# CaNS-World/CaLES

Measured on AMD Instinct MI355X. Metric: time-steps/sec, higher is better.
Workload: dtype f64; 1 GPU; turbulent channel 512x512x512, sgstype=dsmag, PP/PP/NN pressure BCs, bulk forcing in x (BASELINE.json configs[2]); 3 RK substeps/step; decomposition=single GPU

## Files before the change

cales_amd/csrc/api.hip:

```cpp
#include "common.hpp"

static thread_local std::string g_create_err;

void launch_failed(cales_ctx *c, const char *what, hipError_t e) {
  if (c->launch_err.empty()) c->launch_err = std::string("kernel launch failed: ") + what + ": " + hipGetErrorString(e) + " (the context is unusable from here on)";
}
static int finish_pending(cales_ctx *c);
#define ENTER(c) do { LAUNCHCHK(c); if (const int pe_ = finish_pending(c)) return pe_; } while (0)
#define ENTRY(c, expr) do { ENTER(c); const int e_ = (expr); if (e_) return e_; LAUNCHCHK(c); return 0; } while (0)

int stream_after(cales_ctx *c, hipStream_t later, hipStream_t earlier) {
  if (c->sync_ev.size() < 64) { hipEvent_t e; HIPCHK(c, hipEventCreateWithFlags(&e, hipEventDisableTiming)); c->sync_ev.push_back(e); c->sync_next = c->sync_ev.size() - 1; }
  hipEvent_t e = c->sync_ev[c->sync_next]; c->sync_next = (c->sync_next + 1) % c->sync_ev.size();
  HIPCHK(c, hipEventRecord(e, earlier));
  HIPCHK(c, hipStreamWaitEvent(later, e, 0));
  return 0;
}
int prof_begin(cales_ctx *c, const char *name, hipStream_t s) {
  int slot = -1;
  for (size_t q = 0; q < c->stats.size(); ++q) if (c->stats[q].name == name) { slot = (int)q; break; }
  if (slot < 0) { KernelStat s; s.name = name; c->stats.push_back(s); slot = (int)c->stats.size() - 1; }
  std::pair<hipEvent_t, hipEvent_t> ev;
  if (!c->evpool.empty()) { ev = c->evpool.back(); c->evpool.pop_back(); }
  else { hipEventCreate(&ev.first); hipEventCreate(&ev.second); }
  hipEventRecord(ev.first, s ? s : c->stream);
  c->pending.push_back({slot, ev});
  return (int)c->pending.size() - 1;
}
void prof_end(cales_ctx *c, int idx, hipStream_t s) { hipEventRecord(c->pending[idx].second.second, s ? s : c->stream); }
void prof_flush(cales_ctx *c) {
  if (c->pending.empty()) return;
  hipStreamSynchronize(c->stream);
  if (c->comm_stream) hipStreamSynchronize(c->comm_stream);
  for (auto &pe : c->pending) {
    float ms = 0.f;
    hipEventElapsedTime(&ms, pe.second.first, pe.second.second);
    c->stats[pe.first].calls += 1; c->stats[pe.first].ms += ms;
    c->evpool.push_back(pe.second);
  }
  c->pending.clear();
}

static int dev_alloc(cales_ctx *c, real **p, size_t n, bool zero = true) {
  HIPCHK(c, hipMalloc(p, (n ? n : 1) * sizeof(real)));
  if (zero) HIPCHK(c, hipMemset(*p, 0, (n ? n : 1) * sizeof(real)));
  return 0;
}
static int field_alloc(cales_ctx *c, real **p) {
  real *base = nullptr;
  if (dev_alloc(c, &base, c->ntot + LINE_REALS)) return 1;
  *p = base + c->field_ofs;
  return 0;
}
static void field_free(cales_ctx *c, real *p) { if (p) hipFree(p - c->field_ofs); }
static int field_alloc_multi(cales_ctx *c, int k, real **p) {
  real *base = nullptr;
  const size_t one = c->ntot + LINE_REALS;
  if (dev_alloc(c, &base, (size_t)k * one)) return 1;
  for (int q = 0; q < k; ++q) p[q] = base + (size_t)q * one + c->field_ofs;
  c->pp_companion_bytes = one * sizeof(real); c->comp_one = one;
  return 0;
// ... 106 lines not shown
  for (int d = 0; d < 3; ++d) { c->dl[d] = cs->l[d] / (real)(1.f * (float)cs->ng[d]); c->dli[d] = 1. / c->dl[d]; }
  c->visc = 1. / cs->visci;
  Geom &g = c->g;
  g.n1 = c->n[0]; g.n2 = c->n[1]; g.n3 = c->n[2];
  g.s1 = (g.n1 + 3 + LINE_REALS - 1) / LINE_REALS * LINE_REALS;
  c->field_ofs = LINE_REALS - 1;
  g.s12 = (long)g.s1 * (g.n2 + 2); g.jlo = c->lo[1] - 1; g.ng2 = cs->ng[1];
  c->ntot = (size_t)g.s12 * (g.n3 + 2);
  const int n3 = c->n[2];
  c->dzc.resize(n3 + 2); c->dzf.resize(n3 + 2); c->zc.resize(n3 + 2); c->zf.resize(n3 + 2);
  c->dzci.resize(n3 + 2); c->dzfi.resize(n3 + 2); c->gvr_c.resize(n3 + 2); c->gvr_f.resize(n3 + 2);
  hs_initgrid(cs->gtype, n3, cs->gr, cs->l[2], c->dzc.data(), c->dzf.data(), c->zc.data(), c->zf.data());
  for (int k = 0; k <= n3 + 1; ++k) {
    c->dzci[k] = 1. / c->dzc[k]; c->dzfi[k] = 1. / c->dzf[k];
    c->gvr_c[k] = c->dl[0] * c->dl[1] * c->dzc[k] / (cs->l[0] * cs->l[1] * cs->l[2]);
    c->gvr_f[k] = c->dl[0] * c->dl[1] * c->dzf[k] / (cs->l[0] * cs->l[1] * cs->l[2]);
  }
  if (upload_vec(c, &c->d_dzc, c->dzc) || upload_vec(c, &c->d_dzf, c->dzf) || upload_vec(c, &c->d_zc, c->zc) || upload_vec(c, &c->d_zf, c->zf) ||
      upload_vec(c, &c->d_dzci, c->dzci) || upload_vec(c, &c->d_dzfi, c->dzfi) || upload_vec(c, &c->d_gvr_c, c->gvr_c) || upload_vec(c, &c->d_gvr_f, c->gvr_f))
    return fail(5);
  c->is_bound[0] = c->is_bound[1] = 1;
  { c->is_bound[2] = (!c->per_y && r == 0) ? 1 : 0; c->is_bound[3] = (!c->per_y && r == P - 1) ? 1 : 0;
    const bool per_z = cs->cbcpre[4] == 'P' && cs->cbcpre[5] == 'P';
    c->is_bound[4] = c->is_bound[5] = per_z ? 0 : 1; }
  std::vector<real> hb[11][3];
  hs_initbc(c, hb);
  for (int q = 0; q < 11; ++q) if (upload_bound(c, *bs[q], hb[q])) return fail(6);
  for (int d = 1; d <= 3; ++d) for (int s = 0; s <= 1; ++s) c->is_wall[s + 2 * (d - 1)] = (ISB(c, s, d) && CBV(c, s, d, d) == 'D') ? 1. : 0.;
  for (int s = 0; s <= 1; ++s) c->is_wall[s + 2] = (!c->per_y && CBV(c, s, 2, 2) == 'D') ? 1. : 0.;
  sgs_setup(c);
  bc_setup(c);
  { const int *n = c->n;
    const real dx01[2] = {c->dl[0], c->dl[0]}, dy01[2] = {c->dl[1], c->dl[1]};
    const real dzc01[2] = {c->dzc[0], c->dzc[n3]}, dzf01[2] = {c->dzf[1], c->dzf[n3]};
    std::vector<real> rx((size_t)n[1] * n[2] * 2), ry((size_t)n[0] * n[2] * 2), rz((size_t)n[0] * n[1] * 2);
    hs_bc_rhs(&cs->cbcpre[0], hb[3][0].data(), n[1], n[2], dx01, dx01, 'c', rx.data());
    hs_bc_rhs(&cs->cbcpre[2], hb[3][1].data(), n[0], n[2], dy01, dy01, 'c', ry.data());
    hs_bc_rhs(&cs->cbcpre[4], hb[3][2].data(), n[0], n[1], dzc01, dzf01, 'c', rz.data());
    if (upload_vec(c, &c->rhsbp[0], rx) || upload_vec(c, &c->rhsbp[1], ry) || upload_vec(c, &c->rhsbp[2], rz)) return fail(7); }
  const int nfields = cs->impdiff ? CALES_NFIELDS : CALES_DUDTD;
  c->vel_comp = P > 1 && fold_correc_possible(c) && c->n[1] >= 4 && 3 * (c->ntot + 2 * LINE_REALS) * sizeof(real) < (1ull << 32) && !c->fl.unmerged_bc;
  for (int q = 0; q < nfields; ++q) {
    if (q == CALES_PP) continue;
    if (c->vel_comp && q <= CALES_W) { real *two[2]; if (field_alloc_multi(c, 2, two)) return fail(8); c->f[q] = two[0]; }
    else if (field_alloc(c, &c->f[q])) return fail(8);
  }
  { real *three[3]; if (field_alloc(c, &c->scr1) || field_alloc_multi(c, c->vel_comp ? 3 : 2, three)) return fail(9);
    c->f[CALES_PP] = three[0]; c->scr2 = three[1]; c->scr3 = c->vel_comp ? three[2] : nullptr; }
  for (int q = 0; q < 3; ++q) {
    if (c->vel_comp) { real *two[2]; if (field_alloc_multi(c, 2, two)) return fail(9); c->f2[q] = two[0]; }
    else if (field_alloc(c, &c->f2[q])) return fail(9);
  }
  c->red_blocks = 8;
  if (dev_alloc(c, &c->d_red, 64 + 16 * (size_t)(n3 + 2) + 6 * (size_t)(n3 + 2)) || dev_alloc(c, &c->d_force, 8)) return fail(10);
  c->res = c->d_red;
  if (hipHostMalloc((void **)&c->h_red, 64 * sizeof(real)) != hipSuccess) { c->err = "hipHostMalloc failed"; return fail(11); }
  if (cs->sgstype >= 1) {
    if (field_alloc(c, &c->s0)) return fail(12);
    const int nw = cs->sgstype == 1 ? 3 : 6;
    for (int m = 0; m < nw; ++m) if (field_alloc(c, &c->wk[m])) return fail(12);
  }
  if (cs->sgstype == 2) {
    if (field_alloc(c, &c->uc) || field_alloc(c, &c->vc) || field_alloc(c, &c->wc) || field_alloc(c, &c->uf) ||
        field_alloc(c, &c->vf) || field_alloc(c, &c->wf) || field_alloc(c, &c->alph2) || dev_alloc(c, &c->d_p1d, 2 * (size_t)n3 + 2))
      return fail(13);
    if (c->sgs.pair) {
      for (int m = 0; m < 3; ++m) { real *b = nullptr; if (dev_alloc(c, &b, 2 * c->ntot + 2 * LINE_REALS)) return fail(13); c->ss2[m] = b + 2 * c->field_ofs; }
    } else
    for (int m = 0; m < 6; ++m) if (field_alloc(c, &c->sij[m]) || field_alloc(c, &c->mij[m])) return fail(13);
  }
  if (solver_setup(c)) return fail(14);
  { hipDeviceProp_t pr; int dev = 0; if (hipGetDevice(&dev) == hipSuccess && hipGetDeviceProperties(&pr, dev) == hipSuccess) c->ncu = pr.multiProcessorCount; }
  if (sgs_setup_launches(c)) return fail(14);
  mom_setup(c);
  if (hipStreamSynchronize(c->stream) != hipSuccess) { c->err = "sync failed"; return fail(15); }
  if (!c->launch_err.empty()) { c->err = c->launch_err; return fail(16); }
  *out = c;
  return 0;
}

int cales_sync(cales_ctx *c) { ENTER(c); HIPCHK(c, hipStreamSynchronize(c->stream)); return 0; }
int cales_local_size(const cales_ctx *c, int32_t n[3], int32_t lo[3]) { for (int d = 0; d < 3; ++d) { n[d] = c->n[d]; lo[d] = c->lo[d]; } return 0; }

int cales_set_field(cales_ctx *c, int field, const real *host) {
  ENTER(c);
  if (field < 0 || field >= CALES_NFIELDS || !c->f[field]) { c->err = "bad field id"; return 1; }
  if (field == CALES_VISCT) { c->visct_zero = false; c->visct_lazy = false; }
  const size_t nh = (size_t)(c->n[0] + 2) * (c->n[1] + 2) * (c->n[2] + 2);
  const dim3 b(64, 4, 1), gr((c->n[0] + 2 + 63) / 64, (c->n[1] + 2 + 3) / 4, c->n[2] + 2);
  HIPCHK(c, hipMemcpyAsync(c->scr1, host, nh * sizeof(real), hipMemcpyHostToDevice, c->stream));
  LAUNCH(c, k_repack, gr, b, 0, c->stream, c->g, 1, c->f[field], c->scr1);
  LAUNCHCHK(c);
  HIPCHK(c, hipStreamSynchronize(c->stream));
  return 0;
}
int cales_get_field(cales_ctx *c, int field, real *host) {
  ENTER(c);
  if (field < 0 || field >= CALES_NFIELDS || !c->f[field]) { c->err = "bad field id"; return 1; }
  if (field == CALES_VISCT) if (int e = materialize_visct(c)) return e;
  const size_t nh = (size_t)(c->n[0] + 2) * (c->n[1] + 2) * (c->n[2] + 2);
  const dim3 b(64, 4, 1), gr((c->n[0] + 2 + 63) / 64, (c->n[1] + 2 + 3) / 4, c->n[2] + 2);
  LAUNCH(c, k_repack, gr, b, 0, c->stream, c->g, 0, c->f[field], c->scr1);
  LAUNCHCHK(c);
  HIPCHK(c, hipMemcpyAsync(host, c->scr1, nh * sizeof(real), hipMemcpyDeviceToHost, c->stream));
  HIPCHK(c, hipStreamSynchronize(c->stream));
  return 0;
}
// ... 144 lines not shown
  pl.any_wm = any_wm(c);
  pl.fuse_fill = fuse_fill_possible(c) && solver_can_fuse_fillps(c);
  pl.xskip = pl.fuse_fill && xskip_possible(c);
  pl.fold_correc = pl.xskip && fold_correc_possible(c) && (c->P == 1 || c->comm.on);
  pl.fold_rows2 = pl.fold_correc && c->vel_comp;
  pl.fold_mom = !pl.fold_correc && fold_mom_ok(c);
  pl.lazy_last = pl.fold_mom && !fl.eager_projection && c->P == 1 && (fl.lazy_projection || (size_t)c->n[0] * c->n[1] * c->n[2] >= ((size_t)1 << 22));
  { const char *bz = &c->cbcvel[4];
    pl.defer_imp_rhs = c->C.impdiff == 2 && !fl.helmholtz_z_per_column && !fl.unfused_imp_rhs &&
                       !(bz[0] == 'P' && bz[1] == 'P') && !(bz[6] == 'P' && bz[7] == 'P') && !(bz[12] == 'P' && bz[13] == 'P'); }
  { bool dead = !wm_samples_ghost(c);
    for (int sd = 0; sd <= 1; ++sd) if (LWM(c, sd, 1) != 0) dead = false;
    pl.skip_first_wm = dead && pl.any_wm && !fl.unmerged_bc; }
  pl.fuse_cu = fuse_cu_possible(c);
  { bool ok = c->C.impdiff == 0 && pl.fuse_cu && !fl.unfused_forcing && (!pl.any_wm || pl.skip_first_wm);
    for (int d = 0; d < 3; ++d) if (c->C.is_forced[d]) ok = ok && c->cbcvel[6 * d + 2 * d] == 'P' && c->cbcvel[6 * d + 2 * d + 1] == 'P';
    pl.force_mask = (c->C.is_forced[0] ? 1 : 0) | (c->C.is_forced[1] ? 2 : 0) | (c->C.is_forced[2] ? 4 : 0);
    pl.defer_force = ok && pl.force_mask != 0; }
  pl.mean_mask = (pl.fuse_fill && pl.defer_force && !fl.unfused_mean) ? pl.force_mask : 0;
  pl.keep_last_rhs = fl.keep_last_rhs;
  pl.visct_ghosts = !(c->C.sgstype == 0 && (c->visct_zero || c->sgs_first));
  for (int q = 0; q < 6; ++q) if (c->C.bcsgs[q] != 0.) pl.visct_ghosts = true;
  c->plan = pl;
}
static const StepPlan &current_plan(cales_ctx *c) {
  const StepPlan &pl = c->plan;
  if (!pl.valid || pl.in_visct_zero != c->visct_zero || pl.in_sgs_first != c->sgs_first || pl.in_comm_on != c->comm.on || pl.in_overlap != (c->comm_stream != nullptr)) make_plan(c);
  return c->plan;
}
int cales_describe_plan(cales_ctx *c, char *buf, int buflen) {
  if (!c || !buf || buflen < 1) return 1;
  const StepPlan &pl = current_plan(c);
  std::string s;
  s += std::string("projection=") + (pl.fold_rows2 ? "in_strain_rate_pass(ghost_rows_local)" : pl.fold_correc ? "in_strain_rate_pass" : pl.fold_mom ? (pl.lazy_last ? "in_next_momentum_pass(all_substeps)" : "in_next_momentum_pass(substeps_1_2)") : (pl.fuse_cu ? "own_pass(correc+updatep)" : "own_passes"));
  s += std::string(";x_ghost_columns=") + (pl.xskip ? "wrapped" : "maintained");
  s += std::string(";fillps=") + (pl.fuse_fill ? "in_x_transform" : "own_pass");
  s += std::string(";bulk_forcing=") + (pl.force_mask == 0 ? "none" : pl.defer_imp_rhs ? "in_helmholtz_sweep" : pl.defer_force ? (pl.mean_mask ? "in_correction(means_in_x_transform)" : "in_correction(means_own_pass)") : "own_pass");
  if (c->C.impdiff == 2) s += std::string(";implicit_rhs=") + (pl.defer_imp_rhs ? "in_helmholtz_sweep" : "own_pass");
  if (pl.any_wm) s += std::string(";first_wall_model_update=") + (pl.skip_first_wm ? "skipped" : "kept");
  s += std::string(";ghost_cells=") + (c->fl.unmerged_bc ? "by_direction" : "one_launch");
  s += std::string(";visct_ghost_cells=") + (pl.visct_ghosts ? "updated" : "zero_field");
  s += std::string(";momentum=") + (c->mom.fused ? "fused_mom_rk" : "mom+rk_update");
  s += std::string(";sgs=") + sgs_path_name(c);
  s += std::string(";solver=") + solver_path_name(c);
  if (c->P > 1) s += ";mode_columns_per_rank=" + std::to_string(solver_mode_columns(c));
  s += ";ranks=" + std::to_string(c->P) + ";exchanges=" + (c->P == 1 ? "none" : !c->comm.on ? "unset" : (c->comm_stream && (c->comm.halo_s || c->comm.a2a_part)) ? "second_stream" : "in_order");
  std::snprintf(buf, buflen, "%s", s.c_str());
  return (int)s.size() < buflen ? 0 : 2;
}

static int step_body(cales_ctx *c, real dt);
int cales_step(cales_ctx *c, real dt) {
  LAUNCHCHK(c);
  const int e = step_body(c, dt);
  LAUNCHCHK(c);
  if (e) { c->launch_err = "an earlier cales_step failed (" + c->err + "): the fields are in an intermediate state, the context is unusable"; return e; }
  return 0;
}
static int step_body(cales_ctx *c, real dt) {
  static const real rk[3][2] = {{32. / 60., 0.}, {25. / 60., -17. / 60.}, {45. / 60., -25. / 60.}};
  const StepPlan pl = current_plan(c);
  if (c->pend.dtrk != 0. && !pl.fold_mom) { if (int e = finish_pending(c)) return e; }
  PendingProjection pend = c->pend;
  c->pend = PendingProjection();
  LAUNCH(c, k_zero6, dim3(1), dim3(64), 0, c->stream, c->d_force, pend.dtrk != 0. ? 3 : 0);
  c->in_step = true;
  StepMode mode{c};
  if (c->pend_xrefresh && !pl.xskip) {
    c->pend_xrefresh = false; c->step_xskip = true;
    if (int e = end_of_step_refresh(c)) return e;
  }
  c->step_xskip = pl.xskip;
  const int fmask = pl.defer_force ? pl.force_mask : 0;
  SgsFold fold{0., pl.fold_rows2, fmask};
  for (int irk = 1; irk <= 3; ++irk) {
    const real dtrk = (rk[irk - 1][0] + rk[irk - 1][1]) * dt, dtrki = 1. / dtrk;
    real alpha = 0.;
    const bool p_ghosts_due = pend.dtrk != 0. && !pend.p_done;
    { RkOpts o; o.mean_mask = pl.mean_mask; o.rhs_in_sweep = pl.defer_imp_rhs; o.store_rhs = irk < 3 || pl.keep_last_rhs; o.pending = pend.dtrk != 0. ? &pend : nullptr;
      if (int e = op_rk(c, irk, dt, o)) return e;
      pend = PendingProjection(); }
    if (!pl.defer_force && !pl.defer_imp_rhs) { if (int e = op_bulk_forcing(c)) return e; }
    if (c->C.impdiff == 2) {
      alpha = -.5 * c->visc * dtrk;
      const real hf12 = .5 * (rk[irk - 1][0] * dt + rk[irk - 1][1] * dt);
      for (int iv = 1; iv <= 3; ++iv) if (int e = op_helmholtz_z(c, iv, alpha, pl.defer_imp_rhs, hf12)) return e;
    } else if (c->C.impdiff == 1) {
      alpha = -.5 * c->visc * dtrk;
      for (int iv = 1; iv <= 3; ++iv) if (int e = op_helmholtz(c, iv, alpha)) return e;
    }
    { BcCall b; b.skip_wm = pl.skip_first_wm;
      if (p_ghosts_due) b.rider(c->f[CALES_P], 0);
      HaloBatch rows; if (pl.fold_rows2) b.collect = &rows;
      if (int e = op_bounduvw(c, c->bcu, c->bcv, c->bcw, 1, 0, c->f[CALES_U], c->f[CALES_V], c->f[CALES_W], b)) return e;
      if (pl.fold_rows2) {
        if (int e = halo_y_rows(c, 3, c->f + CALES_U, 2, b)) return e;
        if (int e = halo_flush_deferred(c, rows, false)) return e;
      } }
    if (!pl.fuse_fill) { if (int e = op_fillps(c, dtrki)) return e; if (int e = op_updt_rhs_b(c)) return e; }
    if (int e = op_solver(c, pl.fuse_fill ? FusedFill{dtrki, pl.mean_mask} : FusedFill())) return e;
    if (pl.fold_rows2) {
      HaloBatch rows; BcCall b; b.collect = &rows;
      real *one[1] = {c->f[CALES_PP]};
      if (int e = op_boundp(c, c->f[CALES_PP], 0, b)) return e;
      if (int e = halo_y_rows(c, 1, one, 2, b)) return e;
      if (int e = halo_y_rows(c, 1, one, 3, b)) return e;
// ... 128 lines not shown
```

cales_amd/csrc/common.hpp:

```cpp
#pragma once
#include <hip/hip_runtime.h>
#include <cstdint>
#include <cstdio>
#include <cstdlib>
#include <cstring>
#include <cmath>
#include <string>
#include <vector>
#include "../../include/cales.h"

typedef cales_real real;
#ifdef CALES_SINGLE
typedef float2 real2;
#define CALES_EPS 1.1920929e-07f
#define CALES_BIG 3.4028235e38f
#else
typedef double2 real2;
#define CALES_EPS 2.220446049250313e-16
#define CALES_BIG 1.7976931348623157e308
#endif
constexpr int RSZ = (int)sizeof(real);
constexpr int LINE_REALS = 128 / RSZ;
__host__ __device__ inline real2 make_real2(real x, real y) { real2 r; r.x = x; r.y = y; return r; }

struct Geom {
  int n1, n2, n3;
  int s1;
  long s12;
  int jlo;
  int ng2;

  __host__ __device__ inline size_t ix(int i, int j, int k) const { return (size_t)i + (size_t)s1 * (size_t)j + (size_t)s12 * (size_t)k; }
};

struct DBound { real *x, *y, *z; };
struct RhsBz {
  const real *bc; char ctype, cf; real dlc, dlf, sgn, alpha;
  __host__ __device__ inline real at(int i, int j, int n1) const {
    const real bcv = bc[i + (size_t)(n1 + 2) * j];
    real r = 0.;
    if (cf == 'c') { if (ctype == 'D') r = -2. * bcv / dlc / dlf; else if (ctype == 'N') r = sgn * bcv / dlf; }
    else           { if (ctype == 'D') r = -bcv / dlc / dlf;      else if (ctype == 'N') r = sgn * bcv / dlc; }
    return r * alpha;
  }
};

struct Comm {
  cales_halo_cb halo = nullptr; cales_alltoall_cb a2a = nullptr; cales_allreduce_cb allred = nullptr; void *user = nullptr;
  real *A = nullptr, *B = nullptr; int64_t nbuf = 0;
  bool on = false;
  cales_halo_s_cb halo_s = nullptr; cales_alltoall_part_cb a2a_part = nullptr;
};

struct Spec {
  int blocked, cw, n2l, n3;
  int nyq = 0;
  __host__ __device__ inline size_t at_slab(const Geom &g, int m, int jl, int k) const {
    if (!blocked) return (g.ix(0, jl, k) >> 1) + (size_t)m;
    const int peer = m / cw, mm = m - peer * cw;
    return (size_t)mm + (size_t)cw * ((size_t)(jl - 1) + (size_t)n2l * ((size_t)(k - 1) + (size_t)n3 * peer));
  }
  __host__ __device__ inline size_t at_mode(const Geom &g, int mm, int j, int k) const {
    if (!blocked) return (g.ix(0, j, k) >> 1) + (size_t)mm;
    const int peer = (j - 1) / n2l, jl = (j - 1) - peer * n2l;
    return (size_t)mm + (size_t)cw * ((size_t)jl + (size_t)n2l * ((size_t)(k - 1) + (size_t)n3 * peer));
  }
};

struct Flags {
  bool unfolded_correc = false, unfolded_mom = false, eager_projection = false, lazy_projection = false, helmholtz_z_per_column = false, unfused_imp_rhs = false, unfused_correc = false, unfused_forcing = false, unfused_fillps = false, unfused_mean = false, keep_last_rhs = false, wide_offsets = false, dsmag_reference_sequence = false, dsmag_xghosts = false, smag_reference_sequence = false, gaussel_march = false, fft_generic = false, fft_no_odd_radix = false, keep_null_mode = false, unfused_rk = false, overlap = false, xghosts_in_step = false, unmerged_bc = false, no_nyquist_packing = false;
  int kchunk = 0; long tile_min_blocks = 2048;
  std::string test_bad_launch;
  void read_env() {
    test_bad_launch = getenv("CALES_TEST_BAD_LAUNCH") ? getenv("CALES_TEST_BAD_LAUNCH") : "";
    unfolded_mom = getenv("CALES_UNFOLDED_MOM") != nullptr;
    lazy_projection = getenv("CALES_LAZY_PROJECTION") != nullptr;
    eager_projection = getenv("CALES_EAGER_PROJECTION") != nullptr;
    unfolded_correc = getenv("CALES_UNFOLDED_CORREC") != nullptr;
    helmholtz_z_per_column = getenv("CALES_HELMHOLTZ_Z_PER_COLUMN") != nullptr;
    unfused_imp_rhs = getenv("CALES_UNFUSED_IMP_RHS") != nullptr;
    unfused_correc = getenv("CALES_UNFUSED_CORREC") != nullptr;
    unfused_forcing = getenv("CALES_UNFUSED_FORCING") != nullptr;
    unfused_fillps = getenv("CALES_UNFUSED_FILLPS") != nullptr;
    unfused_mean = getenv("CALES_UNFUSED_MEAN") != nullptr;
    keep_last_rhs = getenv("CALES_KEEP_LAST_RHS") != nullptr;
    wide_offsets = getenv("CALES_WIDE_OFFSETS") != nullptr;
    dsmag_reference_sequence = getenv("CALES_DSMAG_REFERENCE_SEQUENCE") != nullptr;
    dsmag_xghosts = getenv("CALES_DSMAG_XGHOSTS") != nullptr;
    smag_reference_sequence = getenv("CALES_SMAG_REFERENCE_SEQUENCE") != nullptr;
    gaussel_march = getenv("CALES_GAUSSEL_MARCH") != nullptr;
    no_nyquist_packing = getenv("CALES_NO_NYQUIST_PACKING") != nullptr;
    fft_generic = getenv("CALES_FFT_GENERIC") != nullptr;
    fft_no_odd_radix = getenv("CALES_FFT_NO_ODD_RADIX") != nullptr;
    xghosts_in_step = getenv("CALES_XGHOSTS_IN_STEP") != nullptr;
    keep_null_mode = getenv("CALES_KEEP_NULL_MODE") != nullptr;
    unfused_rk = getenv("CALES_UNFUSED_RK") != nullptr;
    overlap = getenv("CALES_OVERLAP") != nullptr && atoi(getenv("CALES_OVERLAP")) != 0 && getenv("CALES_NO_OVERLAP") == nullptr;
    unmerged_bc = getenv("CALES_UNMERGED_BC") != nullptr;
    kchunk = getenv("CALES_KCHUNK") ? atoi(getenv("CALES_KCHUNK")) : 0;
    tile_min_blocks = getenv("CALES_TILE_MIN_BLOCKS") ? atol(getenv("CALES_TILE_MIN_BLOCKS")) : 2048;
  }
};

struct StepPlan {
  bool valid = false;
  bool in_visct_zero = false, in_sgs_first = false, in_comm_on = false, in_overlap = false;
  bool xskip = false;
  bool fold_correc = false;
  bool fold_rows2 = false;
  bool fold_mom = false;
  bool lazy_last = false;
  bool defer_imp_rhs = false;
  bool any_wm = false, skip_first_wm = false;
  bool fuse_cu = false;
  bool defer_force = false;
  bool fuse_fill = false;
  bool visct_ghosts = false;
  bool keep_last_rhs = false;
  int mean_mask = 0, force_mask = 0;
};

struct BandMap { int gx, gy, gz, sub; };
struct TileGeom { dim3 block, grid; int kchunk = 0; BandMap bm{0, 0, 0, 0}; };

enum class SgsForm { none, smag_rows, smag_reference, dsmag_tiles, dsmag_reference };
enum class StrainKernel { corr_rows2, corr, yw32, yw64, pair, plain32, plain64 };
enum class LmfKernel { pair, yw_ucf32, yw_ucf64, yw32, yw64, ucf32, ucf64, plain32, plain64 };
enum class SmagKernel { yw32, yw64, plain32, plain64 };
struct SgsPath {
  SgsForm form = SgsForm::none;
  bool pair = false, lazy = false, ucf = false, small = false, yw = false;
  bool wraps_x = true;
  int zlo = 0, zhi = 0, wmlo = 0, wmhi = 0, wylo = 0, wyhi = 0, wmylo = 0, wmyhi = 0; real flo = 0., fhi = 0.;
  int perz = 0, perx = 0, skipz = 0, lmf_ty = 0;
  StrainKernel strain = StrainKernel::plain64; LmfKernel lmf = LmfKernel::plain64; SmagKernel smag = SmagKernel::plain64;
  TileGeom strain_geo, corr_geo, corr_rows2_geo, lmf_geo, smag_geo;
};
struct SgsFold { real dtrk; bool rows2; int fmask; };

struct MomPath {
  bool fused = true;
  int imp = 0;
  bool small = false;
  TileGeom geo;
  bool wm = false, wm_ghosts_in_step = false;
};
struct PendingProjection { real dtrk = 0.; int fmask = 0; bool p_done = false, xskip = false; };

enum class BcForm { merged, all, by_direction };
struct BcPath {
  BcForm vel = BcForm::by_direction, wm = BcForm::by_direction, cell[2] = {BcForm::by_direction, BcForm::by_direction};
// ... 14 lines not shown
struct FusedFill { real dtrki = 0.; int mean_mask = 0; };

struct KernelStat { std::string name; int64_t calls = 0; real ms = 0.; };
struct Solver;

struct cales_ctx {
  cales_case C;
  Flags fl;
  StepPlan plan;
  Geom g;
  int n[3], lo[3];
  real dl[3], dli[3], visc;
  hipStream_t stream; bool own_stream;
  hipStream_t comm_stream = nullptr;
  std::vector<hipEvent_t> sync_ev; size_t sync_next = 0;
  std::string err;
  std::string launch_err;
  std::vector<real> dzc, dzf, zc, zf, dzci, dzfi, gvr_c, gvr_f;
  char cbcvel[18];
  int is_bound[6], index_wm[6];
  real *d_dzc, *d_dzf, *d_zc, *d_zf, *d_dzci, *d_dzfi, *d_gvr_c, *d_gvr_f;
  real *f[CALES_NFIELDS];
  real *f2[3] = {nullptr, nullptr, nullptr};
  size_t ntot;
  DBound bcu, bcv, bcw, bcp, bcs, bcuf, bcvf, bcwf, bcu_mag, bcv_mag, bcw_mag;
  real *rhsbp[3];
  real *rhsbz_vel;
  Solver *solver = nullptr;
  real *d_a, *d_b, *d_c;
  real *d_av[3], *d_bv[3], *d_cv[3];
  real *scr1, *scr2;
  real *d_red; real *h_red;
  real *d_force;
  int red_blocks;
  real *ss2[3] = {nullptr, nullptr, nullptr};
  real *s0, *wk[6], *sij[6], *mij[6], *uc, *vc, *wc, *uf, *vf, *wf, *alph2, *d_p1d;
  real is_wall[6];
  SgsPath sgs;
  BcPath bc;
  MomPath mom;
  bool sgs_first;
  int P = 1, rank = 0; bool per_y = true; int cw = 0;
  Comm comm;
  bool p1d_in_comm = false;
  real *res = nullptr;
  bool prof = false;
  std::vector<KernelStat> stats;
  std::vector<std::pair<int, std::pair<hipEvent_t, hipEvent_t>>> pending;
  std::vector<std::pair<hipEvent_t, hipEvent_t>> evpool;
  real *d_del = nullptr;
  void *native_comm = nullptr;
  bool visct_zero = true;
  bool visct_lazy = false; real *d_cs = nullptr;
  bool in_step = false;
  real *d_stat2 = nullptr;
  real *d_stat = nullptr;
  bool abct_ready = false, force_zeroed = false;
  real *d_abct = nullptr;
  struct HzTab { real alpha = 0.; int nz = 0; bool ok = false; } hz_tab[3][4]; int hz_next[3] = {0, 0, 0}; real *d_hztab = nullptr;
  int ncu = 0;
  real *d_mpart = nullptr; size_t n_mpart = 0;
  bool step_xskip = false;
  PendingProjection pend;
  bool pend_xrefresh = false;
  size_t pp_companion_bytes = 0;
  bool vel_comp = false; size_t comp_one = 0; real *scr3 = nullptr;
  int field_ofs = 0;
  real *d_nullw = nullptr;
};

#define CBV(c, side, dir, vel) ((c)->cbcvel[(side) + 2 * ((dir) - 1) + 6 * ((vel) - 1)])
#define CBP(c, side, dir) ((c)->C.cbcpre[(side) + 2 * ((dir) - 1)])
#define CBS(c, side, dir) ((c)->C.cbcsgs[(side) + 2 * ((dir) - 1)])
#define LWM(c, side, dir) ((c)->C.lwm[(side) + 2 * ((dir) - 1)])
#define ISB(c, side, dir) ((c)->is_bound[(side) + 2 * ((dir) - 1)])
#define IWM(c, side, dir) ((c)->index_wm[(side) + 2 * ((dir) - 1)])

#define HIPCHK(ctx, call)                                                                          \
  do {                                                                                             \
    hipError_t e_ = (call);                                                                        \
    if (e_ != hipSuccess) {                                                                        \
      (ctx)->err = std::string(#call) + ": " + hipGetErrorString(e_);                              \
      return 1;                                                                                    \
    }                                                                                              \
  } while (0)

void launch_failed(cales_ctx *c, const char *what, hipError_t e);
#define LAUNCH(c, kernel, grid, block, lds, stream, ...)                                           \
  do {                                                                                             \
    dim3 blk_ = (block);                                                                           \
    if (!(c)->fl.test_bad_launch.empty() && strstr(#kernel, (c)->fl.test_bad_launch.c_str())) blk_ = dim3(4096, 1, 1); \
    hipLaunchKernelGGL(kernel, grid, blk_, lds, stream, __VA_ARGS__);                              \
    const hipError_t le_ = hipGetLastError();                                                      \
    if (le_ != hipSuccess) launch_failed(c, #kernel, le_);                                         \
  } while (0)
#define LAUNCHCHK(c)                                                                               \
  do {                                                                                             \
    if (!(c)->launch_err.empty()) { (c)->err = (c)->launch_err; return 1; }                        \
  } while (0)
#define HIPSOFT(c, call)                                                                           \
  do {                                                                                             \
    const hipError_t e_ = (call);                                                                  \
    if (e_ != hipSuccess) launch_failed(c, #call, e_);                                             \
  } while (0)

int  prof_begin(cales_ctx *c, const char *name, hipStream_t s = nullptr);
// ... 157 lines not shown
```

cales_amd/csrc/k_stencil.hip:

```cpp
#include "common.hpp"

#define BX 64
#define BY 4

__constant__ real c_rk[3][2] = {{32. / 60., 0.}, {25. / 60., -17. / 60.}, {45. / 60., -25. / 60.}};

template <int IMP>
__global__ __launch_bounds__(BX *BY) void k_mom(Geom g, const real *__restrict__ u, const real *__restrict__ v,
                                                 const real *__restrict__ w, const real *__restrict__ s,
                                                 const real *__restrict__ dzci, const real *__restrict__ dzfi, real dxi,
                                                 real dyi, real visc, real *__restrict__ dudt, real *__restrict__ dvdt,
                                                 real *__restrict__ dwdt, real *__restrict__ dudtd,
                                                 real *__restrict__ dvdtd, real *__restrict__ dwdtd) {
  int bx_, by_, bz_; stencil_block(bx_, by_, bz_);
  const int i = bx_ * BX + threadIdx.x + 1, j = by_ * BY + threadIdx.y + 1, k = bz_ + 1;
  if (i > g.n1 || j > g.n2) return;
  const size_t c = g.ix(i, j, k);
  const long sj = g.s1, sk = g.s12;
#define LD(a, di, dj, dk) a[c + (di) + (dj)*sj + (dk)*sk]
  const real u_ccm = LD(u, 0, 0, -1), u_cmc = LD(u, 0, -1, 0),
               u_mcc = LD(u, -1, 0, 0), u_ccc = LD(u, 0, 0, 0), u_pcc = LD(u, 1, 0, 0), u_mpc = LD(u, -1, 1, 0),
               u_cpc = LD(u, 0, 1, 0), u_mcp = LD(u, -1, 0, 1), u_ccp = LD(u, 0, 0, 1);
  const real v_ccm = LD(v, 0, 0, -1), v_cmc = LD(v, 0, -1, 0), v_pmc = LD(v, 1, -1, 0),
               v_mcc = LD(v, -1, 0, 0), v_ccc = LD(v, 0, 0, 0), v_pcc = LD(v, 1, 0, 0), v_cpc = LD(v, 0, 1, 0),
// ... 317 lines not shown
  const size_t c = g.ix(side ? g.n1 + 1 : 0, j, k);
  const real pc = pp[c];
  if (!side) u[c] = u[c] - fi * (pp[c + 1] - pc);
  if (j <= g.n2) v[c] = v[c] - fj * (pp[c + g.s1] - pc);
  if (k <= g.n3) w[c] = w[c] - dt * dzci[k] * (pp[c + g.s12] - pc);
}
int op_correc_updatep(cales_ctx *c, real dt, real alpha, int upd, int fmask) {
  ProfScope ps(c, upd ? "correc_updatep" : "correc");
  const int *n = c->n;
  dim3 b(BX, BY, 1), gr((n[0] + BX - 1) / BX, (n[1] + 2 + BY - 1) / BY, n[2] + 2);
  real *f_[4] = {c->f[CALES_U], c->f[CALES_V], c->f[CALES_W], c->f[CALES_P]};
  const real fi = dt * c->dli[0], fj = dt * c->dli[1];
  const int mode = !upd ? 0 : (c->C.impdiff == 2 ? 2 : 1);
  const int perx = c->step_xskip ? 1 : 0;
  const auto k_correc_cell_mode = mode == 0 ? k_correc_cell<0> : mode == 1 ? k_correc_cell<1> : k_correc_cell<2>;
  LAUNCH(c, k_correc_cell_mode, gr, b, 0, c->stream, c->g, fi, fj, dt, alpha, c->d_dzci, c->d_dzfi, c->f[CALES_PP], f_[0], f_[1], f_[2], f_[3], c->d_force, fmask, perx);
  if (!(c->in_step && c->cbcvel[0] == 'P' && c->cbcvel[1] == 'P'))
    LAUNCH(c, k_correc_edge, dim3((n[1] + 2 + 63) / 64, (n[2] + 2 + 3) / 4, 2), dim3(64, 4, 1), 0, c->stream, c->g, fi, fj, dt, c->d_dzci, c->f[CALES_PP],
                       f_[0], f_[1], f_[2]);
  LAUNCHCHK(c);
  return 0;
}
int op_correc(cales_ctx *c, real dt, int fmask) {
  if (!c->fl.unfused_correc) return op_correc_updatep(c, dt, 0., 0, fmask);
  ProfScope ps(c, "correc");
  dim3 b(BX, BY, 1), gr = grid3(c->n[0] + 2, c->n[1] + 2, c->n[2] + 2, b);
  LAUNCH(c, k_correc, gr, b, 0, c->stream, c->g, dt * c->dli[0], dt * c->dli[1], dt, c->d_dzci, c->f[CALES_PP], c->f[CALES_U],
                     c->f[CALES_V], c->f[CALES_W]);
  LAUNCHCHK(c);
  return 0;
}

template <int IMP>
__global__ __launch_bounds__(BX *BY) void k_updatep(Geom g, real alpha, real dxi, real dyi, const real *__restrict__ dzci,
                                                     const real *__restrict__ dzfi, const real *__restrict__ pp, real *__restrict__ p) {
  const int i = blockIdx.x * BX + threadIdx.x + 1, j = blockIdx.y * BY + threadIdx.y + 1, k = blockIdx.z + 1;
  if (i > g.n1 || j > g.n2) return;
  const size_t c = g.ix(i, j, k);
  if (IMP == 0) p[c] = p[c] + pp[c];
  else if (IMP == 1)
    p[c] = p[c] + pp[c] + alpha * ((pp[c + 1] - 2. * pp[c] + pp[c - 1]) * (dxi * dxi) + (pp[c + g.s1] - 2. * pp[c] + pp[c - g.s1]) * (dyi * dyi) +
                                   ((pp[c + g.s12] - pp[c]) * dzci[k] - (pp[c] - pp[c - g.s12]) * dzci[k - 1]) * dzfi[k]);
  else p[c] = p[c] + pp[c] + alpha * (((pp[c + g.s12] - pp[c]) * dzci[k] - (pp[c] - pp[c - g.s12]) * dzci[k - 1]) * dzfi[k]);
}
int op_updatep(cales_ctx *c, real alpha) {
  ProfScope ps(c, "updatep");
  dim3 b(BX, BY, 1), gr = grid3(c->n[0], c->n[1], c->n[2], b);
  const auto k_updatep_imp = c->C.impdiff == 2 ? k_updatep<2> : c->C.impdiff == 1 ? k_updatep<1> : k_updatep<0>;
  LAUNCH(c, k_updatep_imp, gr, b, 0, c->stream, c->g, alpha, c->dli[0], c->dli[1], c->d_dzci, c->d_dzfi, c->f[CALES_PP], c->f[CALES_P]);
  LAUNCHCHK(c);
  return 0;
}

__global__ __launch_bounds__(256) void k_chkdiv_partial(Geom g, real dxi, real dyi, const real *__restrict__ dzfi,
                                                        const real *__restrict__ u, const real *__restrict__ v,
                                                        const real *__restrict__ w, real *__restrict__ psum, real *__restrict__ pmax) {
  __shared__ real sh[4];
  const int k = blockIdx.y + 1;
  real acc = 0., mx = 0.;
  for (int j = blockIdx.x * 4 + threadIdx.y + 1; j <= g.n2; j += gridDim.x * 4)
  for (int i = threadIdx.x + 1; i <= g.n1; i += 64) {
    const size_t c = g.ix(i, j, k);
    const real div = (w[c] - w[c - g.s12]) * dzfi[k] + (v[c] - v[c - g.s1]) * dyi + (u[c] - u[c - 1]) * dxi;
    mx = fmax(mx, fabs(div)); acc += div;
  }
  const real rs = block_reduce<0>(acc, sh), rm = block_reduce<1>(mx, sh);
  if (threadIdx.x == 0 && threadIdx.y == 0) { const size_t o = (size_t)blockIdx.y * gridDim.x + blockIdx.x; psum[o] = rs; pmax[o] = rm; }
}
int op_chkdiv(cales_ctx *c, real *divtot, real *divmax) {
  const int nbx = 8, np = nbx * c->n[2];
  LAUNCH(c, k_chkdiv_partial, dim3(nbx, c->n[2]), dim3(64, 4), 0, c->stream, c->g, c->dli[0], c->dli[1], c->d_dzfi, c->f[CALES_U],
                     c->f[CALES_V], c->f[CALES_W], c->d_red + 64, c->d_red + 64 + np);
  LAUNCH(c, k_fold, dim3(1), dim3(256), 0, c->stream, c->d_red + 64, np, 0, c->res, 0);
  LAUNCH(c, k_fold, dim3(1), dim3(256), 0, c->stream, c->d_red + 64 + np, np, 1, c->res, 1);
  if (int e = allreduce_res(c, 0, 1, 0)) return e;
  if (int e = allreduce_res(c, 1, 1, 1)) return e;
  HIPCHK(c, hipMemcpyAsync(c->h_red, c->res, 2 * sizeof(real), hipMemcpyDeviceToHost, c->stream));
  HIPCHK(c, hipStreamSynchronize(c->stream));
  *divtot = c->h_red[0]; *divmax = c->h_red[1];
  return 0;
}

#define NSTAT 27
__global__ __launch_bounds__(256) void k_stats_chan_partial(Geom g, real dx, real dy, const real *__restrict__ dzc, const real *__restrict__ dzf,
                                                            const real *__restrict__ u, const real *__restrict__ v, const real *__restrict__ w,
                                                            const real *__restrict__ p, const real *__restrict__ s, real *__restrict__ part) {
  __shared__ real sh[4];
  const int k = blockIdx.y + 1;
  real b[NSTAT];
#pragma unroll
  for (int q = 0; q < NSTAT; ++q) b[q] = 0.;
  const long nplane = (long)g.n1 * g.n2, sj = g.s1, sk = g.s12;
  const real zc = dzc[k], zfp = dzf[k + 1], zf = dzf[k];
  for (long q = (long)blockIdx.x * 256 + threadIdx.x; q < nplane; q += (long)gridDim.x * 256) {
    const int i = (int)(q % g.n1) + 1, j = (int)(q / g.n1) + 1;
    const size_t c = g.ix(i, j, k);
    const real uc = u[c], vc = v[c], wc = w[c], pc = p[c];
    const real u_kp = u[c + sk], u_ip = u[c + 1], u_im = u[c - 1], u_jp = u[c + sj];
    const real v_kp = v[c + sk], v_ip = v[c + 1], v_jp = v[c + sj], v_jm = v[c - sj];
    const real w_ip = w[c + 1], w_jp = w[c + sj], w_kp = w[c + sk], w_km = w[c - sk];
    b[0] += uc; b[1] += vc; b[2] += wc;
    b[3] += uc * uc; b[4] += vc * vc; b[5] += wc * wc;
    b[6] += 0.25 * (u_kp + uc) * (wc + w_ip);
    b[7] += uc * uc * uc; b[8] += vc * vc * vc; b[9] += wc * wc * wc;
    b[10] += (uc * uc) * (uc * uc); b[11] += (vc * vc) * (vc * vc); b[12] += (wc * wc) * (wc * wc);
    b[13] += pc; b[14] += pc * pc;
    const real ox = (w_jp - wc) / dy - (v_kp - vc) / zc, oy = (u_kp - uc) / zc - (w_ip - wc) / dx, oz = (v_ip - vc) / dx - (u_jp - uc) / dy;
    b[15] += ox; b[16] += oy; b[17] += oz; b[18] += ox * ox; b[19] += oy * oy; b[20] += oz * oz;
    const real s_ccc = s[c], s_pcc = s[c + 1], s_cpc = s[c + sj], s_ccp = s[c + sk], s_pcp = s[c + 1 + sk];
    const real dudx_ip = (u_ip - uc) / dx, dudx_im = (uc - u_im) / dx, dvdy_jp = (v_jp - vc) / dy, dvdy_jm = (vc - v_jm) / dy;
    const real dwdz_kp = (w_kp - wc) / zfp, dwdz_km = (wc - w_km) / zf, dudz = (u_kp - uc) / zc, dwdx = (w_ip - wc) / dx;
    b[21] -= 0.5 * (s_pcc * (dudx_ip + dudx_ip) + s_ccc * (dudx_im + dudx_im));
    b[22] -= 0.5 * (s_cpc * (dvdy_jp + dvdy_jp) + s_ccc * (dvdy_jm + dvdy_jm));
    b[23] -= 0.5 * (s_ccp * (dwdz_kp + dwdz_kp) + s_ccc * (dwdz_km + dwdz_km));
    b[24] -= 0.25 * (s_ccc + s_pcc + s_ccp + s_pcp) * (dudz + dwdx);
    b[25] += s_ccc;
    b[26] += dudz;
  }
#pragma unroll
  for (int q = 0; q < NSTAT; ++q) {
    const real r = block_reduce<0>(b[q], sh);
    if (threadIdx.x == 0) part[((size_t)blockIdx.y * gridDim.x + blockIdx.x) * NSTAT + q] = r;
// ... 178 lines not shown
  return 0;
}
__global__ __launch_bounds__(256) void k_out1d_chan(Geom g, real ratio, const real *__restrict__ u, const real *__restrict__ v, const real *__restrict__ w, real *__restrict__ out) {
  __shared__ real sh[4];
  const int k = blockIdx.x + 1;
  real b[7] = {0., 0., 0., 0., 0., 0., 0.};
  const long np = (long)g.n1 * g.n2, sk = g.s12;
  for (long q = threadIdx.x; q < np; q += 256) {
    const size_t c = g.ix((int)(q % g.n1) + 1, (int)(q / g.n1) + 1, k);
    const real uc = u[c], vc = v[c], wc = w[c], wm = w[c - sk];
    b[0] += uc; b[1] += vc; b[2] += 0.50 * (wm + wc);
    b[3] += uc * uc; b[4] += vc * vc; b[5] += 0.50 * (wc * wc + wm * wm);
    b[6] += 0.25 * (u[c - 1] + uc) * (wm + wc);
  }
#pragma unroll
  for (int q = 0; q < 7; ++q) { const real r = block_reduce<0>(b[q], sh); if (threadIdx.x == 0) out[q + 7 * (size_t)(k - 1)] = r * ratio; }
}
int op_out1d_chan(cales_ctx *c, real *buf) {
  const int n3 = c->n[2];
  real *out = nullptr; HIPCHK(c, hipMalloc(&out, (size_t)7 * n3 * sizeof(real)));
  LAUNCH(c, k_out1d_chan, dim3(n3), dim3(256), 0, c->stream, c->g, c->dl[0] * c->dl[1] / (c->C.l[0] * c->C.l[1]), c->f[CALES_U], c->f[CALES_V], c->f[CALES_W], out);
  LAUNCHCHK(c);
  HIPCHK(c, hipMemcpyAsync(buf, out, (size_t)7 * n3 * sizeof(real), hipMemcpyDeviceToHost, c->stream));
  HIPCHK(c, hipStreamSynchronize(c->stream));
  hipFree(out);
  return 0;
}
__global__ __launch_bounds__(256) void k_out2d_duct(Geom g, real ratio, const real *__restrict__ u, const real *__restrict__ v, const real *__restrict__ w, real *__restrict__ out) {
  const int lane = threadIdx.x & 63, j = blockIdx.x * 4 + (threadIdx.x >> 6) + 1, k = blockIdx.y + 1;
  if (j > g.n2) return;
  real b[9] = {0., 0., 0., 0., 0., 0., 0., 0., 0.};
  const long sj = g.s1, sk = g.s12;
  for (int i = lane + 1; i <= g.n1; i += 64) {
    const size_t c = g.ix(i, j, k);
    const real uc = u[c], um = u[c - 1], vc = v[c], vm = v[c - sj], wc = w[c], wm = w[c - sk];
    b[0] += uc; b[1] += 0.5 * (vm + vc); b[2] += 0.5 * (wm + wc);
    b[3] += uc * uc; b[4] += 0.5 * (vm * vm + vc * vc); b[5] += 0.5 * (wm * wm + wc * wc);
    b[6] += 0.25 * (um + uc) * (vm + vc); b[7] += 0.25 * (um + uc) * (wm + wc); b[8] += 0.25 * (vm + vc) * (wm + wc);
  }
#pragma unroll
  for (int q = 0; q < 9; ++q) { const real r = wave_sum(b[q]); if (lane == 0) out[q + 9 * ((size_t)(j - 1) + (size_t)g.n2 * (k - 1))] = r * ratio; }
}
int op_out2d_duct(cales_ctx *c, real *buf) {
  const int n2 = c->n[1], n3 = c->n[2];
  real *out = nullptr; HIPCHK(c, hipMalloc(&out, (size_t)9 * n2 * n3 * sizeof(real)));
  LAUNCH(c, k_out2d_duct, dim3((n2 + 3) / 4, n3), dim3(256), 0, c->stream, c->g, c->dl[0] / c->C.l[0], c->f[CALES_U], c->f[CALES_V], c->f[CALES_W], out);
  LAUNCHCHK(c);
  HIPCHK(c, hipMemcpyAsync(buf, out, (size_t)9 * n2 * n3 * sizeof(real), hipMemcpyDeviceToHost, c->stream));
  HIPCHK(c, hipStreamSynchronize(c->stream));
  hipFree(out);
  return 0;
}

template <int IMP>
__global__ __launch_bounds__(256) void k_chkdt_partial(Geom g, real dxi, real dyi, real visc, const real *__restrict__ dzci,
                                                       const real *__restrict__ dzfi, const real *__restrict__ s,
                                                       const real *__restrict__ u, const real *__restrict__ v,
                                                       const real *__restrict__ w, real *__restrict__ pa, real *__restrict__ pd) {
  __shared__ real sh[4];
  const int k = blockIdx.y + 1;
  const real dl2i = dxi * dxi + dyi * dyi, zf2 = dzfi[k] * dzfi[k], zc2 = dzci[k] * dzci[k];
  real dti = 0., dtid = 0.;
  const long sj = g.s1, sk = g.s12;
  for (int j = blockIdx.x * 4 + threadIdx.y + 1; j <= g.n2; j += gridDim.x * 4)
  for (int i = threadIdx.x + 1; i <= g.n1; i += 64) {
    const size_t c = g.ix(i, j, k);
    const real ux = fabs(u[c]), vx = 0.25 * fabs(v[c] + v[c - sj] + v[c + 1] + v[c + 1 - sj]),
                 wx = 0.25 * fabs(w[c] + w[c - sk] + w[c + 1] + w[c + 1 - sk]);
    const real uy = 0.25 * fabs(u[c] + u[c + sj] + u[c - 1 + sj] + u[c - 1]), vy = fabs(v[c]),
                 wy = 0.25 * fabs(w[c] + w[c + sj] + w[c + sj - sk] + w[c - sk]);
    const real uz = 0.25 * fabs(u[c] + u[c - 1] + u[c - 1 + sk] + u[c + sk]), vz = 0.25 * fabs(v[c] + v[c - sj] + v[c - sj + sk] + v[c + sk]),
                 wz = fabs(w[c]);
    const real dtix = ux * dxi + vx * dyi + wx * dzfi[k], dtiy = uy * dxi + vy * dyi + wy * dzfi[k], dtiz = uz * dxi + vz * dyi + wz * dzci[k];
    dti = fmax(fmax(fmax(dti, dtix), dtiy), dtiz);
    const real viscx = 0.5 * (s[c] + s[c + 1]), viscy = 0.5 * (s[c] + s[c + sj]), viscz = 0.5 * (s[c] + s[c + sk]);
    real dtidx = viscx * (dl2i + zf2), dtidy = viscy * (dl2i + zf2), dtidz = viscz * (dl2i + zc2);
    if (IMP != 1) { dtidx += visc * dl2i; dtidy += visc * dl2i; dtidz += visc * dl2i; }
    if (IMP == 0) { dtidx += visc * zf2; dtidy += visc * zf2; dtidz += visc * zc2; }
    dtid = fmax(fmax(fmax(dtid, dtidx), dtidy), dtidz);
  }
  const real ra = block_reduce<1>(dti, sh), rd = block_reduce<1>(dtid, sh);
  if (threadIdx.x == 0 && threadIdx.y == 0) { const size_t o = (size_t)blockIdx.y * gridDim.x + blockIdx.x; pa[o] = ra; pd[o] = rd; }
}
int op_chkdt(cales_ctx *c, real *dtmax) {
  if (int e = materialize_visct(c)) return e;
  const int nbx = 8, np = nbx * c->n[2];
  real **f = c->f;
  const auto k_chkdt_partial_imp = c->C.impdiff == 2 ? k_chkdt_partial<2> : c->C.impdiff == 1 ? k_chkdt_partial<1> : k_chkdt_partial<0>;
  LAUNCH(c, k_chkdt_partial_imp, dim3(nbx, c->n[2]), dim3(64, 4), 0, c->stream, c->g, 1. / c->dl[0], 1. / c->dl[1], c->visc, c->d_dzci,
                     c->d_dzfi, f[CALES_VISCT], f[CALES_U], f[CALES_V], f[CALES_W], c->d_red + 64, c->d_red + 64 + np);
  LAUNCH(c, k_fold, dim3(1), dim3(256), 0, c->stream, c->d_red + 64, np, 1, c->res, 0);
  LAUNCH(c, k_fold, dim3(1), dim3(256), 0, c->stream, c->d_red + 64 + np, np, 1, c->res, 1);
  if (int e = allreduce_res(c, 0, 2, 1)) return e;
  HIPCHK(c, hipMemcpyAsync(c->h_red, c->res, 2 * sizeof(real), hipMemcpyDeviceToHost, c->stream));
  HIPCHK(c, hipStreamSynchronize(c->stream));
  real dti = c->h_red[0], dtid = c->h_red[1];
  if (dti == 0.) dti = 1.;
  if (dtid == 0.) dtid = CALES_EPS;
  *dtmax = std::fmin(0.4125 / dtid, 1.732 / dti);
  return 0;
}
```

Baseline: 27.26 time-steps/s.

## Fuse divergence check into dt check kernel and cache result for next chkdiv

The CFL/dt check kernel now also computes the divergence sum and max in the same pass over u, v, w. The result is stored so that a following op_chkdiv call returns it without launching its own kernel. When the eddy viscosity is lazy, the kernel scales it per plane instead of materializing the full field first. This removes one full-field read pass and the visct materialization at the cost of a heavier kernel and extra validity-tracking state. An env flag keeps the old separate path available.

```diff
diff --git a/cales_amd/csrc/api.hip b/cales_amd/csrc/api.hip
--- a/cales_amd/csrc/api.hip
+++ b/cales_amd/csrc/api.hip
@@ -6,7 +6,7 @@
   if (c->launch_err.empty()) c->launch_err = std::string("kernel launch failed: ") + what + ": " + hipGetErrorString(e) + " (the context is unusable from here on)";
 }
 static int finish_pending(cales_ctx *c);
-#define ENTER(c) do { LAUNCHCHK(c); if (const int pe_ = finish_pending(c)) return pe_; } while (0)
+#define ENTER(c) do { LAUNCHCHK(c); (c)->div_fresh = (c)->div_valid; (c)->div_valid = false; if (const int pe_ = finish_pending(c)) return pe_; } while (0)
 #define ENTRY(c, expr) do { ENTER(c); const int e_ = (expr); if (e_) return e_; LAUNCHCHK(c); return 0; } while (0)
 
 int stream_after(cales_ctx *c, hipStream_t later, hipStream_t earlier) {
@@ -219,7 +219,7 @@
     else if (field_alloc(c, &c->f2[q])) return fail(9);
   }
   c->red_blocks = 8;
-  if (dev_alloc(c, &c->d_red, 64 + 16 * (size_t)(n3 + 2) + 6 * (size_t)(n3 + 2)) || dev_alloc(c, &c->d_force, 8)) return fail(10);
+  if (dev_alloc(c, &c->d_red, 64 + 16 * (size_t)(n3 + 2) + 6 * (size_t)(n3 + 2) + 4 * 8 * (size_t)(n3 + 2)) || dev_alloc(c, &c->d_force, 8)) return fail(10);
   c->res = c->d_red;
   if (hipHostMalloc((void **)&c->h_red, 64 * sizeof(real)) != hipSuccess) { c->err = "hipHostMalloc failed"; return fail(11); }
   if (cs->sgstype >= 1) {
@@ -470,6 +470,7 @@
 static int step_body(cales_ctx *c, real dt);
 int cales_step(cales_ctx *c, real dt) {
   LAUNCHCHK(c);
+  c->div_valid = c->div_fresh = false;
   const int e = step_body(c, dt);
   LAUNCHCHK(c);
   if (e) { c->launch_err = "an earlier cales_step failed (" + c->err + "): the fields are in an intermediate state, the context is unusable"; return e; }
diff --git a/cales_amd/csrc/common.hpp b/cales_amd/csrc/common.hpp
--- a/cales_amd/csrc/common.hpp
+++ b/cales_amd/csrc/common.hpp
@@ -68,7 +68,7 @@
 };
 
 struct Flags {
-  bool unfolded_correc = false, unfolded_mom = false, eager_projection = false, lazy_projection = false, helmholtz_z_per_column = false, unfused_imp_rhs = false, unfused_correc = false, unfused_forcing = false, unfused_fillps = false, unfused_mean = false, keep_last_rhs = false, wide_offsets = false, dsmag_reference_sequence = false, dsmag_xghosts = false, smag_reference_sequence = false, gaussel_march = false, fft_generic = false, fft_no_odd_radix = false, keep_null_mode = false, unfused_rk = false, overlap = false, xghosts_in_step = false, unmerged_bc = false, no_nyquist_packing = false;
+  bool unfolded_correc = false, unfolded_mom = false, eager_projection = false, lazy_projection = false, helmholtz_z_per_column = false, unfused_imp_rhs = false, unfused_correc = false, unfused_forcing = false, unfused_fillps = false, unfused_mean = false, keep_last_rhs = false, wide_offsets = false, dsmag_reference_sequence = false, dsmag_xghosts = false, smag_reference_sequence = false, gaussel_march = false, fft_generic = false, fft_no_odd_radix = false, keep_null_mode = false, unfused_rk = false, overlap = false, xghosts_in_step = false, unmerged_bc = false, no_nyquist_packing = false, separate_checks = false;
   int kchunk = 0; long tile_min_blocks = 2048;
   std::string test_bad_launch;
   void read_env() {
@@ -97,6 +97,7 @@
     unfused_rk = getenv("CALES_UNFUSED_RK") != nullptr;
     overlap = getenv("CALES_OVERLAP") != nullptr && atoi(getenv("CALES_OVERLAP")) != 0 && getenv("CALES_NO_OVERLAP") == nullptr;
     unmerged_bc = getenv("CALES_UNMERGED_BC") != nullptr;
+    separate_checks = getenv("CALES_SEPARATE_CHECKS") != nullptr;
     kchunk = getenv("CALES_KCHUNK") ? atoi(getenv("CALES_KCHUNK")) : 0;
     tile_min_blocks = getenv("CALES_TILE_MIN_BLOCKS") ? atol(getenv("CALES_TILE_MIN_BLOCKS")) : 2048;
   }
@@ -217,6 +218,7 @@
   void *native_comm = nullptr;
   bool visct_zero = true;
   bool visct_lazy = false; real *d_cs = nullptr;
+  bool div_valid = false, div_fresh = false; real div_kept[2] = {0., 0.};
   bool in_step = false;
   real *d_stat2 = nullptr;
   real *d_stat = nullptr;
diff --git a/cales_amd/csrc/k_stencil.hip b/cales_amd/csrc/k_stencil.hip
--- a/cales_amd/csrc/k_stencil.hip
+++ b/cales_amd/csrc/k_stencil.hip
@@ -393,6 +393,14 @@
   return 0;
 }
 
+__device__ inline real cell_div(real dw, real dzfi, real dv, real dyi, real du, real dxi) {
+#pragma clang fp contract(off)
+#ifdef CALES_SINGLE
+  return fma(dv, dyi, dw * dzfi) + du * dxi;
+#else
+  return fma(du, dxi, fma(dw, dzfi, dv * dyi));
+#endif
+}
 __global__ __launch_bounds__(256) void k_chkdiv_partial(Geom g, real dxi, real dyi, const real *__restrict__ dzfi,
                                                         const real *__restrict__ u, const real *__restrict__ v,
                                                         const real *__restrict__ w, real *__restrict__ psum, real *__restrict__ pmax) {
@@ -402,13 +410,14 @@
   for (int j = blockIdx.x * 4 + threadIdx.y + 1; j <= g.n2; j += gridDim.x * 4)
   for (int i = threadIdx.x + 1; i <= g.n1; i += 64) {
     const size_t c = g.ix(i, j, k);
-    const real div = (w[c] - w[c - g.s12]) * dzfi[k] + (v[c] - v[c - g.s1]) * dyi + (u[c] - u[c - 1]) * dxi;
+    const real div = cell_div(w[c] - w[c - g.s12], dzfi[k], v[c] - v[c - g.s1], dyi, u[c] - u[c - 1], dxi);
     mx = fmax(mx, fabs(div)); acc += div;
   }
   const real rs = block_reduce<0>(acc, sh), rm = block_reduce<1>(mx, sh);
   if (threadIdx.x == 0 && threadIdx.y == 0) { const size_t o = (size_t)blockIdx.y * gridDim.x + blockIdx.x; psum[o] = rs; pmax[o] = rm; }
 }
 int op_chkdiv(cales_ctx *c, real *divtot, real *divmax) {
+  if (c->div_fresh) { *divtot = c->div_kept[0]; *divmax = c->div_kept[1]; c->div_valid = true; return 0; }
   const int nbx = 8, np = nbx * c->n[2];
   LAUNCH(c, k_chkdiv_partial, dim3(nbx, c->n[2]), dim3(64, 4), 0, c->stream, c->g, c->dli[0], c->dli[1], c->d_dzfi, c->f[CALES_U],
                      c->f[CALES_V], c->f[CALES_W], c->d_red + 64, c->d_red + 64 + np);
@@ -693,15 +702,21 @@
   return 0;
 }
 
-template <int IMP>
-__global__ __launch_bounds__(256) void k_chkdt_partial(Geom g, real dxi, real dyi, real visc, const real *__restrict__ dzci,
-                                                       const real *__restrict__ dzfi, const real *__restrict__ s,
-                                                       const real *__restrict__ u, const real *__restrict__ v,
-                                                       const real *__restrict__ w, real *__restrict__ pa, real *__restrict__ pd) {
+__device__ inline real plane_scaled(real s, real cs) {
+#pragma clang fp contract(off)
+  return s * cs;
+}
+template <int IMP, int LAZY, int DIV>
+__global__ __launch_bounds__(256) void k_checks_partial(Geom g, real dxi, real dyi, real visc, const real *__restrict__ dzci,
+                                                        const real *__restrict__ dzfi, const real *__restrict__ cs, const real *__restrict__ s,
+                                                        const real *__restrict__ u, const real *__restrict__ v,
+                                                        const real *__restrict__ w, real *__restrict__ pa, real *__restrict__ pd,
+                                                        real *__restrict__ psum, real *__restrict__ pmax) {
   __shared__ real sh[4];
   const int k = blockIdx.y + 1;
   const real dl2i = dxi * dxi + dyi * dyi, zf2 = dzfi[k] * dzfi[k], zc2 = dzci[k] * dzci[k];
-  real dti = 0., dtid = 0.;
+  const real csk = LAZY ? cs[k] : 0., csp = LAZY ? cs[k + 1] : 0.;
+  real dti = 0., dtid = 0., acc = 0., mx = 0.;
   const long sj = g.s1, sk = g.s12;
   for (int j = blockIdx.x * 4 + threadIdx.y + 1; j <= g.n2; j += gridDim.x * 4)
   for (int i = threadIdx.x + 1; i <= g.n1; i += 64) {
@@ -714,27 +729,63 @@
                  wz = fabs(w[c]);
     const real dtix = ux * dxi + vx * dyi + wx * dzfi[k], dtiy = uy * dxi + vy * dyi + wy * dzfi[k], dtiz = uz * dxi + vz * dyi + wz * dzci[k];
     dti = fmax(fmax(fmax(dti, dtix), dtiy), dtiz);
-    const real viscx = 0.5 * (s[c] + s[c + 1]), viscy = 0.5 * (s[c] + s[c + sj]), viscz = 0.5 * (s[c] + s[c + sk]);
+    const real s_c = LAZY ? plane_scaled(s[c], csk) : s[c], s_i = LAZY ? plane_scaled(s[c + 1], csk) : s[c + 1],
+                 s_j = LAZY ? plane_scaled(s[c + sj], csk) : s[c + sj], s_k = LAZY ? plane_scaled(s[c + sk], csp) : s[c + sk];
+    const real viscx = 0.5 * (s_c + s_i), viscy = 0.5 * (s_c + s_j), viscz = 0.5 * (s_c + s_k);
     real dtidx = viscx * (dl2i + zf2), dtidy = viscy * (dl2i + zf2), dtidz = viscz * (dl2i + zc2);
     if (IMP != 1) { dtidx += visc * dl2i; dtidy += visc * dl2i; dtidz += visc * dl2i; }
     if (IMP == 0) { dtidx += visc * zf2; dtidy += visc * zf2; dtidz += visc * zc2; }
     dtid = fmax(fmax(fmax(dtid, dtidx), dtidy), dtidz);
+    if (DIV) {
+      const real div = cell_div(w[c] - w[c - g.s12], dzfi[k], v[c] - v[c - g.s1], dyi, u[c] - u[c - 1], dxi);
+      mx = fmax(mx, fabs(div)); acc += div;
+    }
   }
   const real ra = block_reduce<1>(dti, sh), rd = block_reduce<1>(dtid, sh);
-  if (threadIdx.x == 0 && threadIdx.y == 0) { const size_t o = (size_t)blockIdx.y * gridDim.x + blockIdx.x; pa[o] = ra; pd[o] = rd; }
+  const size_t o = (size_t)blockIdx.y * gridDim.x + blockIdx.x;
+  if (threadIdx.x == 0 && threadIdx.y == 0) { pa[o] = ra; pd[o] = rd; }
+  if (DIV) {
+    const real rs = block_reduce<0>(acc, sh), rm = block_reduce<1>(mx, sh);
+    if (threadIdx.x == 0 && threadIdx.y == 0) { psum[o] = rs; pmax[o] = rm; }
+  }
+}
+__global__ __launch_bounds__(256) void k_fold_each(const real *__restrict__ part, int np, int ops, real *__restrict__ out, int slot) {
+  __shared__ real sh[4];
+  const int op = (ops >> blockIdx.x) & 1;
+  part += (size_t)blockIdx.x * np;
+  real acc = 0.;
+  for (int q = threadIdx.x; q < np; q += 256) acc = op ? fmax(acc, part[q]) : acc + part[q];
+  const real r = op ? block_reduce<1>(acc, sh) : block_reduce<0>(acc, sh);
+  if (threadIdx.x == 0) out[slot + blockIdx.x] = r;
+}
+template <int LAZY, int DIV>
+static void launch_checks(cales_ctx *c, real *part, int nbx) {
+  real **f = c->f; const int np = nbx * c->n[2];
+  const auto k_checks_imp = c->C.impdiff == 2 ? k_checks_partial<2, LAZY, DIV> : c->C.impdiff == 1 ? k_checks_partial<1, LAZY, DIV> : k_checks_partial<0, LAZY, DIV>;
+  LAUNCH(c, k_checks_imp, dim3(nbx, c->n[2]), dim3(64, 4), 0, c->stream, c->g, 1. / c->dl[0], 1. / c->dl[1], c->visc, c->d_dzci,
+                     c->d_dzfi, c->d_cs, f[CALES_VISCT], f[CALES_U], f[CALES_V], f[CALES_W], part, part + np, part + 2 * np, part + 3 * np);
 }
 int op_chkdt(cales_ctx *c, real *dtmax) {
-  if (int e = materialize_visct(c)) return e;
-  const int nbx = 8, np = nbx * c->n[2];
-  real **f = c->f;
-  const auto k_chkdt_partial_imp = c->C.impdiff == 2 ? k_chkdt_partial<2> : c->C.impdiff == 1 ? k_chkdt_partial<1> : k_chkdt_partial<0>;
-  LAUNCH(c, k_chkdt_partial_imp, dim3(nbx, c->n[2]), dim3(64, 4), 0, c->stream, c->g, 1. / c->dl[0], 1. / c->dl[1], c->visc, c->d_dzci,
-                     c->d_dzfi, f[CALES_VISCT], f[CALES_U], f[CALES_V], f[CALES_W], c->d_red + 64, c->d_red + 64 + np);
-  LAUNCH(c, k_fold, dim3(1), dim3(256), 0, c->stream, c->d_red + 64, np, 1, c->res, 0);
-  LAUNCH(c, k_fold, dim3(1), dim3(256), 0, c->stream, c->d_red + 64 + np, np, 1, c->res, 1);
-  if (int e = allreduce_res(c, 0, 2, 1)) return e;
-  HIPCHK(c, hipMemcpyAsync(c->h_red, c->res, 2 * sizeof(real), hipMemcpyDeviceToHost, c->stream));
+  constexpr int nbx = 8; const int np = nbx * c->n[2];
+  if (c->fl.separate_checks) {
+    if (int e = materialize_visct(c)) return e;
+    launch_checks<0, 0>(c, c->d_red + 64, nbx);
+    LAUNCH(c, k_fold, dim3(1), dim3(256), 0, c->stream, c->d_red + 64, np, 1, c->res, 0);
+    LAUNCH(c, k_fold, dim3(1), dim3(256), 0, c->stream, c->d_red + 64 + np, np, 1, c->res, 1);
+    if (int e = allreduce_res(c, 0, 2, 1)) return e;
+  } else {
+    static_assert(nbx == 8, "cales_create sizes d_red for four arrays of 8 n3 partials");
+    real *part = c->d_red + 64 + 22 * (size_t)(c->n[2] + 2);
+    if (c->visct_lazy) launch_checks<1, 1>(c, part, nbx); else launch_checks<0, 1>(c, part, nbx);
+    LAUNCH(c, k_fold_each, dim3(4), dim3(256), 0, c->stream, part, np, 0xb, c->res, 0);
+    if (int e = allreduce_res(c, 0, 2, 1)) return e;
+    if (int e = allreduce_res(c, 2, 1, 0)) return e;
+    if (int e = allreduce_res(c, 3, 1, 1)) return e;
+  }
+  HIPCHK(c, hipMemcpyAsync(c->h_red, c->res, 4 * sizeof(real), hipMemcpyDeviceToHost, c->stream));
   HIPCHK(c, hipStreamSynchronize(c->stream));
+  LAUNCHCHK(c);
+  if (!c->fl.separate_checks) { c->div_kept[0] = c->h_red[2]; c->div_kept[1] = c->h_red[3]; c->div_valid = true; }
   real dti = c->h_red[0], dtid = c->h_red[1];
   if (dti == 0.) dti = 1.;
   if (dtid == 0.) dtid = CALES_EPS;
```

Result: no change. 27.32 time-steps/s (median of 6 runs) (+0.2%).
